# psteinb/libmultiviewnative

Measured on AMD Instinct MI355X. Metric: RL iterations/sec on 512^3 f32, 6 views, higher is better.
Workload: dtype f32

## Files before the change

### libmultiviewnative_amd/csrc/mvn_mid_fused.hpp

```cpp
#pragma once

#include <stdexcept>

#include "mvn_dim0_direct.hpp"
#include "mvn_wave_rows.hpp"

#if defined(__HIPCC__) && !defined(MVN_HOST_EMU)
#define MF_WPHASE(ctx, ...)                                         \
  {                                                                 \
    const int tid = (ctx).tid;                                      \
    auto& r = (ctx).regs;                                           \
    (void)r;                                                        \
    __VA_ARGS__;                                                    \
  }                                                                 \
  __builtin_amdgcn_fence(__ATOMIC_SEQ_CST, "wavefront", "local");   \
  __builtin_amdgcn_wave_barrier();
#else
#define MF_WPHASE(ctx, ...) MVN_PHASE(ctx, __VA_ARGS__)
#endif

#define MF_N1 512
#define MF_NT 512
#define MF_LINES 8
#define MF_PITCH 576
#define MF_BUF (MF_LINES * MF_PITCH)
#define MF_TWL 512
#define MF_LDS_CFLOATS (4 * MF_BUF + MF_TWL)

struct MidFusedParams {
  const cfloat* in;
  cfloat* out;
  const cfloat* taps;
  int kd;
  const cfloat* tw;
  int d0, H;
  int k, h;
  int seg;
  int mode;
  int packed;
  int zbeg, zcount;
  unsigned* poison;
  unsigned poison_epoch;
  int n_peers;
  unsigned* const* poison_peers;
};
enum { MF_CONV = 0, MF_TAPS = 1 };
enum { MF_DC_NONE = 0, MF_DC_LOW = 1, MF_DC_HIGH = 2, MF_DC_SELF = 3 };

constexpr int mf_slots(int K) { return (K + 7) / 8 * 8; }

template <int K>
struct MfRegs {
  cfloat tap[K];
  cfloat w[mf_slots(K)];
  cfloat xr[8];
  cfloat t[8];
  cfloat bad;
  cfloat t2[8];
  cfloat xn[2], xp[2];
  int dcmode, qm, cpar;
};

inline long mf_pieces(const MidFusedParams& P) { return (P.seg > 0 && P.zcount <= 0) ? (P.d0 + P.seg - 1) / P.seg : 1; }
inline long mf_blocks(const MidFusedParams& P) { return P.mode == MF_TAPS ? (long)P.H * ((P.d0 + MF_LINES - 1) / MF_LINES) : (long)P.H * mf_pieces(P); }

MVN_HD void mf_job(const MidFusedParams& P, long block, int& c, int& z0, int& nout) {
  const long piece = block / P.H;
  c = (int)(block - piece * P.H);
  if (P.zcount > 0) {
    z0 = P.zbeg;
    nout = P.zcount;
  } else if (P.seg > 0) {
    z0 = (int)(piece * P.seg);
    nout = P.d0 - z0 < P.seg ? P.d0 - z0 : P.seg;
  } else {
    z0 = 0;
    nout = P.d0;
  }
}

MVN_HD int mf_tap_plane(const MidFusedParams& P, int j) {
  const int p = j - P.h;
  return p < 0 ? p + P.kd : p;
}

#define MVN_MF_TAP_COUNTS(X) X(1) X(3) X(5) X(7) X(9) X(11) X(13) X(15) X(17) X(19) X(21) X(23) X(25) X(27) X(29) X(31)

inline void mf_check(const MidFusedParams& P) {
  const bool taps_mode = P.mode == MF_TAPS;
  if (!P.in || !P.out || !P.tw || P.d0 < 1 || P.H < 1 || (long)P.d0 * P.H * MF_N1 >= (1L << 31) * 4 || P.seg < 0)
    throw std::invalid_argument("mvn: fused middle pass: bad arguments");
  if (P.zcount < 0 || P.zbeg < 0 || P.zbeg + P.zcount > P.d0 || P.n_peers < 0 || P.n_peers > MVN_D0_MAX_PEERS ||
      (P.n_peers > 0 && !P.poison_peers))
    throw std::invalid_argument("mvn: fused middle pass: bad plane range or peers");
  if (!taps_mode && (!P.taps || P.in == P.out || P.k < 1 || mvn_dim0_taps_template(P.k) > 31 || P.h != P.k / 2 || P.kd < P.k))
    throw std::invalid_argument("mvn: fused middle pass called outside its range");
}

MVN_HD int mf_in_plane(const MidFusedParams& P, int z0, int n) {
  int z = (z0 - P.h + n) % P.d0;
  return z < 0 ? z + P.d0 : z;
}

template <int K>
MVN_HD void mf_fetch(const MidFusedParams& P, MfRegs<K>& r, int c, int z0, int batch, int nsteps, int tid) {
  const int wv = tid >> 6, l = tid & 63;
  const int n = batch * MF_LINES + wv;
  if (n >= nsteps) return;
  const cfloat* src = P.in + ((long)mf_in_plane(P, z0, n) * P.H + c) * MF_N1 + l;
#pragma unroll
  for (int m = 0; m < 8; ++m) r.xr[m] = src[64 * m];
}

template <int K>
MVN_HD void mf_setup(const MidFusedParams& P, MfRegs<K>& r, int c, int z0, int nsteps, int tid) {
  r.bad = cmake(0.f, 0.f);
  r.dcmode = MF_DC_NONE;
  r.qm = r.cpar = 0;
#pragma unroll
  for (int j = 0; j < K; ++j) r.tap[j] = j < P.k ? P.taps[((long)mf_tap_plane(P, j) * P.H + c) * MF_N1 + tid] : cmake(0.f, 0.f);
#pragma unroll
  for (int s = 0; s < mf_slots(K); ++s) r.w[s] = cmake(0.f, 0.f);
  mf_fetch<K>(P, r, c, z0, 0, nsteps, tid);
}

MVN_HD cfloat mf_cmul(cfloat a, cfloat w) {
#if defined(MVN_PACKED)
  cfloat t, r;
  MVN_PK2(t, "v_pk_mul_f32", a, w, "op_sel_hi:[0,1]");
  MVN_PK3(r, "v_pk_fma_f32", a, w, t, "op_sel:[1,1,0] op_sel_hi:[1,0,1] neg_lo:[0,1,0]");
  return r;
#else
  return cmul(a, w);
#endif
}
MVN_HD cfloat mf_cmulc(cfloat a, cfloat w) {
#if defined(MVN_PACKED)
  cfloat t, r;
  MVN_PK2(t, "v_pk_mul_f32", a, w, "op_sel_hi:[0,1] neg_hi:[0,1]");
  MVN_PK3(r, "v_pk_fma_f32", a, w, t, "op_sel:[1,1,0] op_sel_hi:[1,0,1]");
  return r;
#else
  return cmulc(a, w);
#endif
}

MVN_HD void mf_build_twiddles(const MidFusedParams& P, cfloat* twl, int tid) {
  if (tid < 448) {
    const int m = tid / 64 + 1, l = tid & 63;
    twl[tid] = P.tw[l * m];
  } else if (tid < 448 + 56) {
    const int e = tid - 448, m = e / 8 + 1, j = e & 7;
    twl[tid] = P.tw[8 * j * m];
  }
}
MVN_HD cfloat mf_tw0(const cfloat* twl, int l, int m) { return twl[(m - 1) * 64 + l]; }
MVN_HD cfloat mf_tw1(const cfloat* twl, int l, int m) { return twl[448 + (m - 1) * 8 + (l & 7)]; }

template <int K>
MVN_HD void mf_fwd0(MfRegs<K>& r, cfloat* buf, int tid) {
  const int wv = tid >> 6, l = tid & 63;
  cfloat* line = buf + wv * MF_PITCH;
  cfloat a[8];
#pragma unroll
  for (int m = 0; m < 8; ++m) a[m] = r.xr[m];
  dftR<8, -1>(a);
#pragma unroll
  for (int m = 1; m < 8; ++m) a[m] = mf_cmul(a[m], r.t2[m]);
#pragma unroll
  for (int m = 0; m < 8; ++m) line[72 * m + l] = a[m];
}
template <int K>
MVN_HD void mf_tw0_ahead(MfRegs<K>& r, const cfloat* twl, int tid) {
  const int l = tid & 63;
#pragma unroll
  for (int m = 1; m < 8; ++m) r.t2[m] = mf_tw0(twl, l, m);
}
template <int K>
MVN_HD void mf_fwd1_r(MfRegs<K>& r, const cfloat* buf, int tid) {
  const int wv = tid >> 6, l = tid & 63;
  const cfloat* p = buf + wv * MF_PITCH + 72 * (l >> 3) + (l & 7);
#pragma unroll
  for (int m = 0; m < 8; ++m) r.t[m] = p[8 * m];
}
template <int K>
MVN_HD void mf_fwd1_c(MfRegs<K>& r, const cfloat* twl, int tid) {
  const int l = tid & 63;
  (void)l;
  dftR<8, -1>(r.t);
#pragma unroll
  for (int m = 1; m < 8; ++m) r.t[m] = mf_cmul(r.t[m], mf_tw1(twl, l, m));
}
template <int K>
MVN_HD void mf_fwd1_r2(MfRegs<K>& r, const cfloat* buf, int tid) {
  const int wv = tid >> 6, l = tid & 63;
  const cfloat* p = buf + wv * MF_PITCH + 72 * (l >> 3) + (l & 7);
#pragma unroll
  for (int m = 0; m < 8; ++m) r.t2[m] = p[8 * m];
}
template <int K>
MVN_HD void mf_fwd1_c2(MfRegs<K>& r, const cfloat* twl, int tid) {
  const int l = tid & 63;
  (void)l;
  dftR<8, -1>(r.t2);
#pragma unroll
  for (int m = 1; m < 8; ++m) r.t2[m] = mf_cmul(r.t2[m], mf_tw1(twl, l, m));
}
template <int K>
MVN_HD void mf_fwd1_b2(const MfRegs<K>& r, cfloat* buf, int tid) {
  const int wv = tid >> 6, l = tid & 63;
  cfloat* p = buf + wv * MF_PITCH + 72 * (l >> 3) + (l & 7);
#pragma unroll
  for (int m = 0; m < 8; ++m) p[9 * m] = r.t2[m];
}
template <int K>
MVN_HD void mf_fwd2_r2(MfRegs<K>& r, const cfloat* buf, int tid) {
  const int wv = tid >> 6, l = tid & 63;
  const cfloat* p = buf + wv * MF_PITCH + 72 * (l >> 3) + 9 * (l & 7);
#pragma unroll
  for (int m = 0; m < 8; ++m) r.t2[m] = p[m];
}
template <int K>
MVN_HD void mf_fwd2_b2(const MfRegs<K>& r, cfloat* buf, int tid) {
  const int wv = tid >> 6, l = tid & 63;
  cfloat* line = buf + wv * MF_PITCH;
#pragma unroll
  for (int m = 0; m < 8; ++m) line[64 * m + l] = r.t2[m];
}
template <int K>
MVN_HD void mf_fwd1_a(MfRegs<K>& r, const cfloat* buf, const cfloat* twl, int tid) {
  mf_fwd1_r<K>(r, buf, tid);
  mf_fwd1_c<K>(r, twl, tid);
}
template <int K>
MVN_HD void mf_fwd1_b(const MfRegs<K>& r, cfloat* buf, int tid) {
  const int wv = tid >> 6, l = tid & 63;
  cfloat* p = buf + wv * MF_PITCH + 72 * (l >> 3) + (l & 7);
#pragma unroll
  for (int m = 0; m < 8; ++m) p[9 * m] = r.t[m];
}
template <int K>
MVN_HD void mf_fwd2_r(MfRegs<K>& r, const cfloat* buf, int tid) {
  const int wv = tid >> 6, l = tid & 63;
  const cfloat* p = buf + wv * MF_PITCH + 72 * (l >> 3) + 9 * (l & 7);
#pragma unroll
  for (int m = 0; m < 8; ++m) r.t[m] = p[m];
}
template <int K>
MVN_HD void mf_fwd2_a(MfRegs<K>& r, const cfloat* buf, int tid) {
  mf_fwd2_r<K>(r, buf, tid);
  dftR<8, -1>(r.t);
}
template <int K>
MVN_HD void mf_fwd2_b(const MfRegs<K>& r, cfloat* buf, int tid) {
  const int wv = tid >> 6, l = tid & 63;
  cfloat* line = buf + wv * MF_PITCH;
#pragma unroll
  for (int m = 0; m < 8; ++m) line[64 * m + l] = r.t[m];
}

template <int K>
MVN_HD void mf_inv2_r(MfRegs<K>& r, const cfloat* buf, int tid) {
  const int wv = tid >> 6, l = tid & 63;
  const cfloat* line = buf + wv * MF_PITCH;
#pragma unroll
  for (int m = 0; m < 8; ++m) r.t[m] = line[64 * m + l];
}
template <int K>
MVN_HD void mf_inv2_a(MfRegs<K>& r, const cfloat* buf, int tid) {
  mf_inv2_r<K>(r, buf, tid);
  dftR<8, +1>(r.t);
}
template <int K>
MVN_HD void mf_inv2_b(const MfRegs<K>& r, cfloat* buf, int tid) {
  const int wv = tid >> 6, l = tid & 63;
  cfloat* p = buf + wv * MF_PITCH + 72 * (l >> 3) + 9 * (l & 7);
#pragma unroll
  for (int m = 0; m < 8; ++m) p[m] = r.t[m];
}
template <int K>
MVN_HD void mf_inv1_r(MfRegs<K>& r, const cfloat* buf, int tid) {
  const int wv = tid >> 6, l = tid & 63;
  const cfloat* p = buf + wv * MF_PITCH + 72 * (l >> 3) + (l & 7);
#pragma unroll
  for (int m = 0; m < 8; ++m) r.t[m] = p[9 * m];
}
template <int K>
MVN_HD void mf_inv1_c(MfRegs<K>& r, const cfloat* twl, int tid) {
  const int l = tid & 63;
  (void)l;
#pragma unroll
  for (int m = 1; m < 8; ++m) r.t[m] = mf_cmulc(r.t[m], mf_tw1(twl, l, m));
  dftR<8, +1>(r.t);
}
template <int K>
MVN_HD void mf_inv1_a(MfRegs<K>& r, const cfloat* buf, const cfloat* twl, int tid) {
  mf_inv1_r<K>(r, buf, tid);
  mf_inv1_c<K>(r, twl, tid);
}
template <int K>
MVN_HD void mf_inv1_b(const MfRegs<K>& r, cfloat* buf, int tid) {
  const int wv = tid >> 6, l = tid & 63;
  cfloat* p = buf + wv * MF_PITCH + 72 * (l >> 3) + (l & 7);
#pragma unroll
  for (int m = 0; m < 8; ++m) p[8 * m] = r.t[m];
}
template <int K>
MVN_HD void mf_inv0_r(MfRegs<K>& r, const cfloat* buf, int tid) {
  const int wv = tid >> 6, l = tid & 63;
  const cfloat* line = buf + wv * MF_PITCH;
#pragma unroll
  for (int m = 0; m < 8; ++m) r.t[m] = line[72 * m + l];
}
template <int K>
MVN_HD void mf_inv0_c_store(MfRegs<K>& r, const cfloat* twl, cfloat* dst, int tid) {
  const int l = tid & 63;
#pragma unroll
  for (int m = 1; m < 8; ++m) r.t[m] = mf_cmulc(r.t[m], mf_tw0(twl, l, m));
  dftR<8, +1>(r.t);
#pragma unroll
  for (int m = 0; m < 8; ++m) dst[l + 64 * m] = r.t[m];
}
template <int K>
MVN_HD void mf_inv0_store(MfRegs<K>& r, const cfloat* buf, const cfloat* twl, cfloat* dst, int tid) {
  mf_inv0_r<K>(r, buf, tid);
  mf_inv0_c_store<K>(r, twl, dst, tid);
}

template <int K>
MVN_HD void mf_store_line(const MidFusedParams& P, MfRegs<K>& r, const cfloat* buf, const cfloat* twl, int c, int z0,
                          int nout, int batch, int tid) {
  const int m = batch * MF_LINES + (tid >> 6) - (K - 1);
  if (m < 0 || m >= nout) return;
  int z = z0 + m;
  z = z >= P.d0 ? z - P.d0 : z;
  mf_inv0_store<K>(r, buf, twl, P.out + ((long)z * P.H + c) * MF_N1, tid);
}
template <int K>
MVN_HD void mf_store_line_c(const MidFusedParams& P, MfRegs<K>& r, const cfloat* twl, int c, int z0, int nout, int batch,
                            int tid) {
  const int m = batch * MF_LINES + (tid >> 6) - (K - 1);
  if (m < 0 || m >= nout) return;
  int z = z0 + m;
  z = z >= P.d0 ? z - P.d0 : z;
  mf_inv0_c_store<K>(r, twl, P.out + ((long)z * P.H + c) * MF_N1, tid);
}

MVN_HD int mf_bin_of(int f) { return 64 * (f >> 6) + 8 * (f & 7) + ((f >> 3) & 7); }
MVN_HD int mf_freq_of(int q) { return ((q >> 3) & 7) + 8 * (q & 7) + 64 * (q >> 6); }
MVN_HD cfloat mf_herm0(cfloat a, cfloat b) { return cmake(0.5f * (a.x + b.x), 0.5f * (a.y - b.y)); }
MVN_HD cfloat mf_hermh(cfloat a, cfloat b) { return cmake(0.5f * (a.y + b.y), 0.5f * (b.x - a.x)); }


template <int K>
MVN_HD void mf_setup_dc(const MidFusedParams& P, MfRegs<K>& r, int tid) {
  const int f = mf_freq_of(tid), fm = (MF_N1 - f) & (MF_N1 - 1);
  r.qm = mf_bin_of(fm);
  r.dcmode = f == fm ? MF_DC_SELF : (f < MF_N1 / 2 ? MF_DC_LOW : MF_DC_HIGH);
  {
    const int l = tid & 63, g = (l >> 3) + 8 * (l & 7);
    r.cpar = g == 0 ? 64 : 8 * ((64 - g) & 7) + ((64 - g) >> 3);
  }
  const cfloat* tp = P.taps + r.qm;
#pragma unroll
  for (int j = 0; j < K; ++j) {
    const cfloat a = r.tap[j], b = j < P.k ? tp[(long)mf_tap_plane(P, j) * P.H * MF_N1] : cmake(0.f, 0.f);
    r.tap[j] = f == fm ? a : (f < MF_N1 / 2 ? mf_herm0(a, b) : mf_hermh(b, a));
  }
}

template <int K>
MVN_HD void mf_fread(MfRegs<K>& r, const cfloat* in, int c, bool dc, int tid) {
  r.xn[c & 1] = in[c * MF_PITCH + tid];
  if (dc) r.xp[c & 1] = in[c * MF_PITCH + r.qm];
}
template <int K>
MVN_HD cfloat mf_filter_input(MfRegs<K>& r, int c, bool dc) {
  cfloat x = r.xn[c & 1];
  if (dc) {
    const cfloat xp = r.xp[c & 1];
    const cfloat lo = mf_herm0(x, xp), hi = mf_hermh(xp, x);
    x = r.dcmode == MF_DC_LOW ? lo : (r.dcmode == MF_DC_HIGH ? hi : x);
  }
  return x;
}
template <int K, int U, int C, bool FILL>
MVN_HD void mf_filter_line(MfRegs<K>& r, const cfloat* in, cfloat* out, bool dc, int tid) {
  constexpr int KW = mf_slots(K), S = 8 * U + C;
  if (FILL) {
    r.w[S] = mf_filter_input<K>(r, C, dc);
    return;
  }
  constexpr int NC = K < 4 ? K : 4;
  cfloat a1[NC], a2[NC];
#pragma unroll
  for (int j = K - 1; j >= 1; --j) {
    const int ch = j % NC;
    const bool first = j + NC > K - 1;
    if (first)
      mvn_cmul2(a1[ch], a2[ch], r.w[(S - j + 2 * KW) % KW], r.tap[j]);
    else
      mvn_cmac2(a1[ch], a2[ch], r.w[(S - j + 2 * KW) % KW], r.tap[j]);
  }
  const cfloat x = mf_filter_input<K>(r, C, dc);
  if (K <= NC)
    mvn_cmul2(a1[0], a2[0], x, r.tap[0]);
  else
    mvn_cmac2(a1[0], a2[0], x, r.tap[0]);
  cfloat s1 = a1[0], s2 = a2[0];
#pragma unroll
  for (int ch = 1; ch < NC; ++ch) {
    s1 = cadd(s1, a1[ch]);
    s2 = cadd(s2, a2[ch]);
  }
  r.w[S] = x;
  r.bad = mvn_dim0_track(r.bad, x);
  cfloat o = cadd_i<+1>(s1, s2);
  if (dc) o = r.dcmode == MF_DC_SELF ? cmake(s1.x, s2.y) : o;
  out[C * MF_PITCH + tid] = o;
}
template <int K, int C>
MVN_HD void mf_fread_ahead(MfRegs<K>& r, const cfloat* in, bool dc, int tid) {
  if (C + 1 < MF_LINES) mf_fread<K>(r, in, C + 1, dc, tid);
}
template <int K, int C, int U>
MVN_HD void mf_fline_dispatch(MfRegs<K>& r, const cfloat* in, cfloat* out, int u, bool fill, bool dc, int tid) {
  if (u == U) {
    if (fill)
      mf_filter_line<K, U, C, true>(r, in, out, dc, tid);
    else
      mf_filter_line<K, U, C, false>(r, in, out, dc, tid);
    return;
  }
  if constexpr (U + 1 < mf_slots(K) / 8) mf_fline_dispatch<K, C, U + 1>(r, in, out, u, fill, dc, tid);
}

template <int K>
MVN_HD void mf_inv2_fix_dc(MfRegs<K>& r, const cfloat* buf, int tid) {
  const int wv = tid >> 6, l = tid & 63;
  const cfloat* line = buf + wv * MF_PITCH;
#pragma unroll
  for (int m = 0; m < 8; ++m) {
    const cfloat o = r.t[m];
    const cfloat p = line[(64 * (7 - m) + r.cpar) & (MF_N1 - 1)];
    const cfloat low = cmake(o.x - p.y, o.y + p.x), high = cmake(p.x + o.y, o.x - p.y);
    cfloat v = m < 4 ? low : high;
    if (m == 0 || m == 4) v = l == 0 ? o : v;
    r.t[m] = v;
  }
}
template <int K>
MVN_HD void mf_inv2_r_dc(MfRegs<K>& r, const cfloat* buf, int tid) {
  mf_inv2_r<K>(r, buf, tid);
  mf_inv2_fix_dc<K>(r, buf, tid);
}

template <int K>
MVN_HD void mf_report(const MidFusedParams& P, const MfRegs<K>& r) {
  if (r.bad.x != 0.f || r.bad.y != 0.f) {
    if (P.poison) *P.poison = P.poison_epoch;
    for (int i = 0; i < P.n_peers; ++i) *P.poison_peers[i] = P.poison_epoch;
  }
}

template <int K, typename Ctx>
MVN_HD void mf_body(const MidFusedParams& P, long block, cfloat* lds, Ctx& ctx) {
  constexpr int NT_ = MF_NT;
  (void)NT_;
  int c, z0, nout;
  mf_job(P, block, c, z0, nout);
  const int nsteps = nout + K - 1;
  const int nb = (nsteps + MF_LINES - 1) / MF_LINES;
  const bool dc = P.packed && c == 0;
  cfloat* twl = lds + 4 * MF_BUF;
  MVN_PHASE_NOSYNC(ctx, (mf_setup<K>(P, r, c, z0, nsteps, tid), mf_build_twiddles(P, twl, tid)));
  if (dc) {
    MVN_PHASE_NOSYNC(ctx, (mf_setup_dc<K>(P, r, tid)));
  }
  MVN_PHASE(ctx, (void)0);
  MVN_PHASE_NOSYNC(ctx, (mf_tw0_ahead<K>(r, twl, tid)));
#if defined(__HIPCC__) && !defined(MVN_HOST_EMU)
  const int wave_young = mvn_uniform((ctx.tid >> 8) & 1);
#define MF_PRIO_RESET() __builtin_amdgcn_s_setprio(0);
#define MF_PRIO_RAISE_YOUNG() \
  if (wave_young != 0) __builtin_amdgcn_s_setprio(2);
#else
#define MF_PRIO_RESET()
#define MF_PRIO_RAISE_YOUNG()
#endif
  for (int i = -1; i <= nb; ++i) {
    const cfloat* fin = lds + (i & 1) * MF_BUF;
    cfloat* fout = lds + (2 + (i & 1)) * MF_BUF;
    cfloat* fwd = lds + ((i + 1) & 1) * MF_BUF;
    cfloat* inv = lds + (2 + ((i + 1) & 1)) * MF_BUF;
    const bool F = i >= 0 && i < nb;
    const bool fill = i * MF_LINES + MF_LINES - 1 < K - 1;
    const int u = F ? i % (mf_slots(K) / 8) : 0;
#define MF_FLINE(C)                                                                \
  if (F) {                                                                         \
    MF_WPHASE(ctx, (mf_fread_ahead<K, C>(r, fin, dc, tid), mf_fline_dispatch<K, C, 0>(r, fin, fout, u, fill, dc, tid)));  \
  }
    MF_PRIO_RESET()
    if (F) {
      MF_WPHASE(ctx, (mf_fread<K>(r, fin, 0, dc, tid)));
    }
    MF_WPHASE(ctx, (mf_inv2_r<K>(r, inv, tid)));
    if (dc) {
      MF_WPHASE(ctx, (mf_inv2_fix_dc<K>(r, inv, tid)));
    }
    MF_WPHASE(ctx, (mf_fwd0<K>(r, fwd, tid), mf_fetch<K>(P, r, c, z0, i + 2, nsteps, tid)));
    MF_FLINE(0)
    MF_WPHASE(ctx, (dftR<8, +1>(r.t), mf_inv2_b<K>(r, inv, tid)));
    MF_WPHASE(ctx, (mf_inv1_r<K>(r, inv, tid)));
    MF_WPHASE(ctx, (mf_fwd1_r2<K>(r, fwd, tid)));
    MF_FLINE(1)
    MF_FLINE(2)
    MF_PRIO_RAISE_YOUNG()
    MF_WPHASE(ctx, (mf_inv1_c<K>(r, twl, tid), mf_inv1_b<K>(r, inv, tid)));
    MF_WPHASE(ctx, (mf_fwd1_c2<K>(r, twl, tid), mf_fwd1_b2<K>(r, fwd, tid)));
    MF_WPHASE(ctx, (mf_inv0_r<K>(r, inv, tid)));
    MF_WPHASE(ctx, (mf_fwd2_r2<K>(r, fwd, tid)));
    MF_FLINE(3)
    MF_FLINE(4)
    MF_WPHASE(ctx, (mf_store_line_c<K>(P, r, twl, c, z0, nout, i - 1, tid)));
    MF_WPHASE(ctx, (dftR<8, -1>(r.t2), mf_fwd2_b2<K>(r, fwd, tid)));
    MF_FLINE(5)
    MF_FLINE(6)
    MF_FLINE(7)
#undef MF_FLINE
    MF_WPHASE(ctx, (mf_tw0_ahead<K>(r, twl, tid)));
    MVN_PHASE(ctx, (void)0);
  }
#undef MF_PRIO_RESET
#undef MF_PRIO_RAISE_YOUNG
  MVN_PHASE_NOSYNC(ctx, (mf_report<K>(P, r)));
}

MVN_HD void mf_taps_load(const MidFusedParams& P, MfRegs<1>& r, long batch, int c, int tid) {
  const int l = tid & 63, z = (int)batch * MF_LINES + (tid >> 6);
  if (z >= P.d0) return;
  const cfloat* src = P.in + ((long)z * P.H + c) * MF_N1 + l;
#pragma unroll
  for (int m = 0; m < 8; ++m) r.xr[m] = src[64 * m];
}
MVN_HD void mf_taps_store(const MidFusedParams& P, const cfloat* lds, long batch, int c, int tid) {
  const int l = tid & 63, wv = tid >> 6, z = (int)batch * MF_LINES + wv;
  if (z >= P.d0) return;
  cfloat* dst = P.out + ((long)z * P.H + c) * MF_N1 + l;
#pragma unroll
  for (int m = 0; m < 8; ++m) dst[64 * m] = lds[wv * MF_PITCH + 64 * m + l];
}
template <typename Ctx>
MVN_HD void mf_taps_body(const MidFusedParams& P, long block, cfloat* lds, Ctx& ctx) {
  constexpr int NT_ = MF_NT;
  (void)NT_;
  const long batch = block / P.H;
  const int c = (int)(block - batch * P.H);
  cfloat* twl = lds + 4 * MF_BUF;
  MVN_PHASE(ctx, (mf_taps_load(P, r, batch, c, tid), mf_build_twiddles(P, twl, tid)));
  MF_WPHASE(ctx, (mf_tw0_ahead<1>(r, twl, tid)));
  MF_WPHASE(ctx, (mf_fwd0<1>(r, lds, tid)));
  MF_WPHASE(ctx, (mf_fwd1_a<1>(r, lds, twl, tid)));
  MF_WPHASE(ctx, (mf_fwd1_b<1>(r, lds, tid)));
  MF_WPHASE(ctx, (mf_fwd2_a<1>(r, lds, tid)));
  MF_WPHASE(ctx, (mf_fwd2_b<1>(r, lds, tid)));
  MVN_PHASE_NOSYNC(ctx, (mf_taps_store(P, lds, batch, c, tid)));
}
```

Baseline: 100.0.

## Peel fill batches into prologue and stream tap loads alongside early batches

The main loop's fill batches and the trailing inverse-only iteration are peeled into a compile-time recursive prologue and an epilogue. This removes the per-iteration F/fill predicates and the empty inverse work in early iterations. Filter tap loads, including the DC Hermitian partner taps staged in unused window slots, are split into groups and issued alongside the prologue's fetch and forward FFT phases, so their global latency overlaps with compute instead of stalling setup. The cost is more code size, some register-pressure risk, and more complex control flow in the first-batch and DC paths.

```diff
diff --git a/libmultiviewnative_amd/csrc/mvn_mid_fused.hpp b/libmultiviewnative_amd/csrc/mvn_mid_fused.hpp
--- a/libmultiviewnative_amd/csrc/mvn_mid_fused.hpp
+++ b/libmultiviewnative_amd/csrc/mvn_mid_fused.hpp
@@ -112,16 +112,31 @@
   for (int m = 0; m < 8; ++m) r.xr[m] = src[64 * m];
 }
 
+constexpr int mf_fill_batches(int K) { return (K - 1) / MF_LINES; }
+constexpr int mf_tap_group(int K) { return (K + mf_fill_batches(K)) / (mf_fill_batches(K) + 1); }
+constexpr int mf_tap_lo(int K, int G) { return G * mf_tap_group(K) < K ? G * mf_tap_group(K) : K; }
+
 template <int K>
 MVN_HD void mf_setup(const MidFusedParams& P, MfRegs<K>& r, int c, int z0, int nsteps, int tid) {
+  mf_fetch<K>(P, r, c, z0, 0, nsteps, tid);
   r.bad = cmake(0.f, 0.f);
   r.dcmode = MF_DC_NONE;
   r.qm = r.cpar = 0;
 #pragma unroll
-  for (int j = 0; j < K; ++j) r.tap[j] = j < P.k ? P.taps[((long)mf_tap_plane(P, j) * P.H + c) * MF_N1 + tid] : cmake(0.f, 0.f);
-#pragma unroll
   for (int s = 0; s < mf_slots(K); ++s) r.w[s] = cmake(0.f, 0.f);
-  mf_fetch<K>(P, r, c, z0, 0, nsteps, tid);
+}
+template <int K, int G>
+MVN_HD void mf_load_taps(const MidFusedParams& P, MfRegs<K>& r, int c, int tid) {
+#pragma unroll
+  for (int j = mf_tap_lo(K, G); j < mf_tap_lo(K, G + 1); ++j)
+    r.tap[j] = j < P.k ? P.taps[((long)mf_tap_plane(P, j) * P.H + c) * MF_N1 + tid] : cmake(0.f, 0.f);
+}
+template <int K>
+MVN_HD void mf_taps_arrived(MfRegs<K>& r) {
+#if defined(__HIPCC__) && !defined(MVN_HOST_EMU)
+#pragma unroll
+  for (int j = 0; j < K; ++j) asm volatile("" : "+v"(r.tap[j]));
+#endif
 }
 
 MVN_HD cfloat mf_cmul(cfloat a, cfloat w) {
@@ -361,11 +376,23 @@
     const int l = tid & 63, g = (l >> 3) + 8 * (l & 7);
     r.cpar = g == 0 ? 64 : 8 * ((64 - g) & 7) + ((64 - g) >> 3);
   }
+}
+template <int K, int G>
+MVN_HD void mf_load_taps_dc(const MidFusedParams& P, MfRegs<K>& r, int tid) {
+  constexpr int S0 = MF_LINES * mf_fill_batches(K), J0 = mf_tap_lo(K, G);
+  static_assert(mf_tap_group(K) <= mf_slots(K) - S0, "a tap group's partner bins fit the window slots the prologue leaves alone");
   const cfloat* tp = P.taps + r.qm;
 #pragma unroll
-  for (int j = 0; j < K; ++j) {
-    const cfloat a = r.tap[j], b = j < P.k ? tp[(long)mf_tap_plane(P, j) * P.H * MF_N1] : cmake(0.f, 0.f);
-    r.tap[j] = f == fm ? a : (f < MF_N1 / 2 ? mf_herm0(a, b) : mf_hermh(b, a));
+  for (int j = J0; j < mf_tap_lo(K, G + 1); ++j)
+    r.w[S0 + j - J0] = j < P.k ? tp[(long)mf_tap_plane(P, j) * P.H * MF_N1] : cmake(0.f, 0.f);
+}
+template <int K, int G>
+MVN_HD void mf_split_taps_dc(MfRegs<K>& r) {
+  constexpr int S0 = MF_LINES * mf_fill_batches(K), J0 = mf_tap_lo(K, G);
+#pragma unroll
+  for (int j = J0; j < mf_tap_lo(K, G + 1); ++j) {
+    const cfloat a = r.tap[j], b = r.w[S0 + j - J0];
+    r.tap[j] = r.dcmode == MF_DC_SELF ? a : (r.dcmode == MF_DC_LOW ? mf_herm0(a, b) : mf_hermh(b, a));
   }
 }
 
@@ -424,15 +451,20 @@
   if (C + 1 < MF_LINES) mf_fread<K>(r, in, C + 1, dc, tid);
 }
 template <int K, int C, int U>
-MVN_HD void mf_fline_dispatch(MfRegs<K>& r, const cfloat* in, cfloat* out, int u, bool fill, bool dc, int tid) {
+MVN_HD void mf_fline_dispatch(MfRegs<K>& r, const cfloat* in, cfloat* out, int u, bool mixed, bool dc, int tid) {
+  constexpr int NU = mf_slots(K) / 8;
   if (u == U) {
-    if (fill)
-      mf_filter_line<K, U, C, true>(r, in, out, dc, tid);
-    else
+    if constexpr (U == mf_fill_batches(K) % NU && C < (K - 1) % MF_LINES) {
+      if (mixed)
+        mf_filter_line<K, U, C, true>(r, in, out, dc, tid);
+      else
+        mf_filter_line<K, U, C, false>(r, in, out, dc, tid);
+    } else {
       mf_filter_line<K, U, C, false>(r, in, out, dc, tid);
+    }
     return;
   }
-  if constexpr (U + 1 < mf_slots(K) / 8) mf_fline_dispatch<K, C, U + 1>(r, in, out, u, fill, dc, tid);
+  if constexpr (U + 1 < NU) mf_fline_dispatch<K, C, U + 1>(r, in, out, u, mixed, dc, tid);
 }
 
 template <int K>
@@ -463,9 +495,40 @@
   }
 }
 
+template <int K, int I, typename Ctx>
+MVN_HD void mf_prologue(const MidFusedParams& P, cfloat* lds, const cfloat* twl, Ctx& ctx, int c, int z0, int nsteps, bool dc) {
+  constexpr int NT_ = MF_NT, U = I < 0 ? 0 : I % (mf_slots(K) / 8);
+  (void)NT_;
+  const cfloat* fin = lds + (I & 1) * MF_BUF;
+  cfloat* fwd = lds + ((I + 1) & 1) * MF_BUF;
+  (void)fin;
+  if constexpr (I >= 0) {
+    if (dc) {
+      MVN_PHASE_NOSYNC(ctx, (mf_split_taps_dc<K, I>(r)));
+    }
+    MF_WPHASE(ctx, (mf_fread<K>(r, fin, 0, dc, tid)));
+  }
+  MF_WPHASE(ctx, (mf_fwd0<K>(r, fwd, tid), mf_fetch<K>(P, r, c, z0, I + 2, nsteps, tid), mf_load_taps<K, I + 1>(P, r, c, tid)));
+  if (dc) {
+    MVN_PHASE_NOSYNC(ctx, (mf_load_taps_dc<K, I + 1>(P, r, tid)));
+  }
+  MF_WPHASE(ctx, (mf_fwd1_r2<K>(r, fwd, tid)));
+  MF_WPHASE(ctx, (mf_fwd1_c2<K>(r, twl, tid), mf_fwd1_b2<K>(r, fwd, tid)));
+  MF_WPHASE(ctx, (mf_fwd2_r2<K>(r, fwd, tid)));
+  MF_WPHASE(ctx, (dftR<8, -1>(r.t2), mf_fwd2_b2<K>(r, fwd, tid)));
+  if constexpr (I >= 0) {
+#define MF_FILL(C) MF_WPHASE(ctx, (mf_fread_ahead<K, C>(r, fin, dc, tid), mf_filter_line<K, U, C, true>(r, fin, nullptr, dc, tid)));
+    MF_FILL(0) MF_FILL(1) MF_FILL(2) MF_FILL(3) MF_FILL(4) MF_FILL(5) MF_FILL(6) MF_FILL(7)
+#undef MF_FILL
+  }
+  MF_WPHASE(ctx, (mf_tw0_ahead<K>(r, twl, tid)));
+  MVN_PHASE(ctx, (void)0);
+  if constexpr (I + 1 < mf_fill_batches(K)) mf_prologue<K, I + 1>(P, lds, twl, ctx, c, z0, nsteps, dc);
+}
+
 template <int K, typename Ctx>
 MVN_HD void mf_body(const MidFusedParams& P, long block, cfloat* lds, Ctx& ctx) {
-  constexpr int NT_ = MF_NT;
+  constexpr int NT_ = MF_NT, MF_P = mf_fill_batches(K);
   (void)NT_;
   int c, z0, nout;
   mf_job(P, block, c, z0, nout);
@@ -479,26 +542,35 @@
   }
   MVN_PHASE(ctx, (void)0);
   MVN_PHASE_NOSYNC(ctx, (mf_tw0_ahead<K>(r, twl, tid)));
+  mf_prologue<K, -1>(P, lds, twl, ctx, c, z0, nsteps, dc);
+  if (dc) {
+    MVN_PHASE_NOSYNC(ctx, (mf_split_taps_dc<K, MF_P>(r)));
+  }
+  MVN_PHASE_NOSYNC(ctx, (mf_taps_arrived<K>(r)));
 #if defined(__HIPCC__) && !defined(MVN_HOST_EMU)
   const int wave_young = mvn_uniform((ctx.tid >> 8) & 1);
 #define MF_PRIO_RESET() __builtin_amdgcn_s_setprio(0);
 #define MF_PRIO_RAISE_YOUNG() \
   if (wave_young != 0) __builtin_amdgcn_s_setprio(2);
+#define MF_OPAQUE(x) asm volatile("" : "+s"(x))
 #else
 #define MF_PRIO_RESET()
 #define MF_PRIO_RAISE_YOUNG()
+#define MF_OPAQUE(x) (void)0
 #endif
-  for (int i = -1; i <= nb; ++i) {
+  int i0 = MF_P, F = 1;
+  MF_OPAQUE(i0);
+  MF_OPAQUE(F);
+  for (int i = i0; i < nb; ++i) {
     const cfloat* fin = lds + (i & 1) * MF_BUF;
     cfloat* fout = lds + (2 + (i & 1)) * MF_BUF;
     cfloat* fwd = lds + ((i + 1) & 1) * MF_BUF;
     cfloat* inv = lds + (2 + ((i + 1) & 1)) * MF_BUF;
-    const bool F = i >= 0 && i < nb;
-    const bool fill = i * MF_LINES + MF_LINES - 1 < K - 1;
-    const int u = F ? i % (mf_slots(K) / 8) : 0;
+    const bool mixed = i == MF_P;
+    const int u = i % (mf_slots(K) / 8);
 #define MF_FLINE(C)                                                                \
   if (F) {                                                                         \
-    MF_WPHASE(ctx, (mf_fread_ahead<K, C>(r, fin, dc, tid), mf_fline_dispatch<K, C, 0>(r, fin, fout, u, fill, dc, tid)));  \
+    MF_WPHASE(ctx, (mf_fread_ahead<K, C>(r, fin, dc, tid), mf_fline_dispatch<K, C, 0>(r, fin, fout, u, mixed, dc, tid)));  \
   }
     MF_PRIO_RESET()
     if (F) {
@@ -533,6 +605,20 @@
   }
 #undef MF_PRIO_RESET
 #undef MF_PRIO_RAISE_YOUNG
+#undef MF_OPAQUE
+  MVN_TILE_LOOP_TOP(ctx);
+  {
+    cfloat* inv = lds + (2 + ((nb + 1) & 1)) * MF_BUF;
+    MF_WPHASE(ctx, (mf_inv2_r<K>(r, inv, tid)));
+    if (dc) {
+      MF_WPHASE(ctx, (mf_inv2_fix_dc<K>(r, inv, tid)));
+    }
+    MF_WPHASE(ctx, (dftR<8, +1>(r.t), mf_inv2_b<K>(r, inv, tid)));
+    MF_WPHASE(ctx, (mf_inv1_r<K>(r, inv, tid)));
+    MF_WPHASE(ctx, (mf_inv1_c<K>(r, twl, tid), mf_inv1_b<K>(r, inv, tid)));
+    MF_WPHASE(ctx, (mf_inv0_r<K>(r, inv, tid)));
+    MF_WPHASE(ctx, (mf_store_line_c<K>(P, r, twl, c, z0, nout, nb - 1, tid)));
+  }
   MVN_PHASE_NOSYNC(ctx, (mf_report<K>(P, r)));
 }
 
```

Result: faster. 101.5, median of 6 (+1.4%).
